# jhuggins/viabel

Measured on AMD Instinct MI355X. Metric: ELBO-gradient evals/sec (D=1024, N_mc=4096), higher is better.
Workload: dtype f64

## Files before the change

viabel_amd/csrc/vb_fullrank.hip:

```cpp
#include "vb_gemm_f64.h"
#include "vb_fit.h"

namespace vb {

constexpr double kLog2PiFr = 1.8378770664093454835606594728112;

__device__ __forceinline__ double fr_wave_sum(double x) {
#pragma unroll
  for (int off = 32; off > 0; off >>= 1) x += __shfl_down(x, off, 64);
  return x;
}

__device__ __forceinline__ double fr_block_sum(double x, double* sh) {
  x = fr_wave_sum(x);
  const int lane = threadIdx.x & 63, wave = threadIdx.x >> 6;
  __syncthreads();
  if (lane == 0) sh[wave] = x;
  __syncthreads();
  return (sh[0] + sh[1]) + (sh[2] + sh[3]);
}

__global__ void __launch_bounds__(256) fr_unpack_kernel(const double* __restrict__ theta, int d,
                                                        int64_t ldl, double* __restrict__ Lt,
                                                        double* __restrict__ mu, double* __restrict__ copy = nullptr) {
// ... 222 lines not shown
    const double v = z[m.k];
    const double w = exp(-2.0 * v);
    const double rw = roww ? roww[row] : 1.0;
    double ss = 0.0;
    for (int c = lane; c < d; c += 64) {
      if (c == m.k) continue;
      const double zc = z[c];
      const double gc = -zc * w;
      g[c] = roww ? gc * rw : gc;
      ss = fma(zc, zc, ss);
    }
    ss = fr_wave_sum(ss);
    if (lane == 0) {
      const double it2 = 1.0 / (m.tau * m.tau), dm1 = (double)(d - 1);
      const double gk = fma(-v, it2, -dm1) + w * ss;
      g[m.k] = roww ? gk * rw : gk;
      f = v * fma(-0.5 * v, it2, -dm1) - 0.5 * w * ss;
    }
  }
  f = fr_block_sum(f, sh);
  if (threadIdx.x == 0) fpart[blockIdx.x] = f;
}

typedef double fr_d2 __attribute__((ext_vector_type(2)));
__global__ void __launch_bounds__(256) fr_colsum_kernel(const double* __restrict__ G,
                                                        const double* __restrict__ Zc, int64_t ldz,
                                                        int64_t n, int d, int fmode,
                                                        const double* __restrict__ ivar,
                                                        double* __restrict__ colpart,
                                                        double* __restrict__ fpart, double scal = 0.0,
                                                        const double* __restrict__ roww = nullptr,
                                                        int square = 0, double* __restrict__ Gscaled = nullptr,
                                                        const double* __restrict__ rs_out = nullptr) {
  __shared__ double sh[4];
  __shared__ fr_d2 cs[4][64];
  const int c = threadIdx.x & 63, q = threadIdx.x >> 6;
  const int col = blockIdx.x * 128 + 2 * c;
  const int64_t r0 = (int64_t)blockIdx.y * 128;
  const int64_t r1 = r0 + 128 < n ? r0 + 128 : n;
  const bool ok0 = col < d, ok1 = col + 1 < d;
  fr_d2 s = (fr_d2){0.0, 0.0};
  double f = 0.0;
  if (ok0) {
    fr_d2 hiv = (fr_d2){0.0, 0.0};
    if (fmode == 1) hiv = (fr_d2){-0.5 / ivar[col], ok1 ? -0.5 / ivar[col + 1] : 0.0};
    for (int64_t rb = r0 + q; rb < r1; rb += 64) {
      fr_d2 g[16], z[16];
      double rw[16], rs[16];
#pragma unroll
      for (int i = 0; i < 16; ++i) {
        const int64_t r = rb + 4 * i < r1 ? rb + 4 * i : r1 - 1;
        g[i] = *reinterpret_cast<const fr_d2*>(G + r * ldz + col);
        z[i] = fmode >= 2 ? *reinterpret_cast<const fr_d2*>(Zc + r * ldz + col) : (fr_d2){0.0, 0.0};
        rw[i] = roww ? roww[r] : 1.0;
        rs[i] = Gscaled ? rs_out[r] : 1.0;
      }
#pragma unroll
      for (int i = 0; i < 16; ++i) {
        const int64_t r = rb + 4 * i;
        const bool in = r < r1;
        if (roww) g[i] *= rw[i];
        if (square) g[i] *= g[i];
        if (!in) g[i] = (fr_d2){0.0, 0.0}, z[i] = (fr_d2){0.0, 0.0};
        if (!ok1) g[i].y = 0.0, z[i].y = 0.0;
        if (Gscaled && in) *reinterpret_cast<fr_d2*>(Gscaled + r * ldz + col) = g[i] * rs[i];
        s += g[i];
        if (fmode == 1) f = fma(hiv.x * g[i].x, g[i].x, fma(hiv.y * g[i].y, g[i].y, f));
        if (fmode == 2) f = fma(0.5 * z[i].x, g[i].x, fma(0.5 * z[i].y, g[i].y, f));
        if (fmode == 3) f = fma(-0.5 * scal * z[i].x, z[i].x, fma(-0.5 * scal * z[i].y, z[i].y, f));
      }
    }
  }
  cs[q][c] = s;
  __syncthreads();
  if (q == 0 && ok0) {
    const fr_d2 tot = (cs[0][c] + cs[1][c]) + (cs[2][c] + cs[3][c]);
    colpart[(int64_t)blockIdx.y * ldz + col] = tot.x;
    if (ok1) colpart[(int64_t)blockIdx.y * ldz + col + 1] = tot.y;
  }
  f = fr_block_sum(f, sh);
  if (threadIdx.x == 0) fpart[(int64_t)blockIdx.y * gridDim.x + blockIdx.x] = f;
}

__global__ void __launch_bounds__(256) fr_fold_ssum_kernel(const double* __restrict__ Spart, int gsplits, int64_t slab, int d,
                                                           int64_t ldl, const double* __restrict__ colpart, int64_t ldz,
                                                           const double* __restrict__ M, const double* __restrict__ P,
                                                           int64_t ldp, const double* __restrict__ mu,
                                                           const double* __restrict__ mean, double n_rows, int nb_cs,
                                                           int nb_s, double* __restrict__ S, double* __restrict__ svec,
                                                           double* __restrict__ b, double* __restrict__ csg) {
  if ((int)blockIdx.x < nb_cs) {
    __shared__ fr_d2 part[2][64][4];
    const int p = threadIdx.x & 3, kg = threadIdx.x >> 2;
    const int col = (int)blockIdx.x * 8 + 2 * p;
    const int colc = col < d ? col : 0;
    const int kper = (d + 63) / 64;
    const int k0 = kg * kper, k1 = k0 + kper < d ? k0 + kper : d;
    fr_d2 acc = (fr_d2){0.0, 0.0}, bacc = (fr_d2){0.0, 0.0};
    for (int kb = k0; kb < k1; kb += 16) {
      fr_d2 v[16];
      double c[16];
#pragma unroll
      for (int u = 0; u < 16; ++u) {
        const int k = kb + u < k1 ? kb + u : k1 - 1;
        v[u] = *reinterpret_cast<const fr_d2*>(P + (int64_t)k * ldp + colc);
        c[u] = mu[k] - mean[k];
      }
#pragma unroll
      for (int u = 0; u < 16; ++u)
        if (kb + u < k1) bacc += v[u] * c[u];
    }
    for (int kb = k0; kb < k1; kb += 16) {
      fr_d2 v[16];
      double c[16];
#pragma unroll
      for (int u = 0; u < 16; ++u) {
        const int k = kb + u < k1 ? kb + u : k1 - 1;
        v[u] = *reinterpret_cast<const fr_d2*>(M + (int64_t)k * ldz + colc);
        c[u] = colpart[k];
      }
      for (int z = 1; z < gsplits; ++z)
#pragma unroll
        for (int u = 0; u < 16; ++u) c[u] += colpart[(int64_t)z * ldz + (kb + u < k1 ? kb + u : k1 - 1)];
#pragma unroll
      for (int u = 0; u < 16; ++u)
        if (kb + u < k1) acc += v[u] * c[u];
    }
    part[0][kg][p] = acc;
    part[1][kg][p] = bacc;
    __syncthreads();
    if (kg == 0) {
      fr_d2 tot = part[0][0][p], btot = part[1][0][p];
#pragma unroll 16
      for (int q = 1; q < 64; ++q) tot += part[0][q][p], btot += part[1][q][p];
      if (col < d) b[col] = btot.x, csg[col] = -tot.x - n_rows * btot.x;
      if (col + 1 < d) b[col + 1] = btot.y, csg[col + 1] = -tot.y - n_rows * btot.y;
    }
    return;
  }
  if ((int)blockIdx.x < nb_cs + nb_s) {
    const int k = ((int)blockIdx.x - nb_cs) * 256 + (int)threadIdx.x;
    if (k >= ldz) return;
    double s = 0.0;
    if (k < d) {
      s = colpart[k];
      for (int z = 1; z < gsplits; ++z) s += colpart[(int64_t)z * ldz + k];
    }
    svec[k] = s;
    return;
  }
  int bi = 0, bj = (int)blockIdx.x - nb_cs - nb_s;
  while (bj > bi) bj -= ++bi;
  __shared__ double tile[32][33];
  const int tx = threadIdx.x & 31, ty = threadIdx.x >> 5;
  const int i0 = bi * 32, j0 = bj * 32;
  double v[4];
  int64_t idx[4];
#pragma unroll
  for (int q = 0; q < 4; ++q) {
    const int i = i0 + ty + 8 * q, j = j0 + tx;
    idx[q] = (i < d && j <= i) ? (int64_t)i * ldl + j : 0;
    v[q] = 0.0;
  }
  for (int zb = 0; zb < gsplits; zb += 8) {
    double w[8][4];
#pragma unroll
    for (int u = 0; u < 8; ++u)
#pragma unroll
      for (int q = 0; q < 4; ++q) w[u][q] = Spart[(zb + u < gsplits ? zb + u : gsplits - 1) * slab + idx[q]];
#pragma unroll
    for (int u = 0; u < 8; ++u)
      if (zb + u < gsplits) {
#pragma unroll
        for (int q = 0; q < 4; ++q) v[q] = (zb + u == 0) ? w[u][q] : v[q] + w[u][q];
      }
  }
#pragma unroll
  for (int q = 0; q < 4; ++q) tile[ty + 8 * q][tx] = v[q];
  __syncthreads();
#pragma unroll
  for (int q = 0; q < 4; ++q) {
    const int r = ty + 8 * q;
    if (bi == bj) {
      const int i = i0 + r, j = j0 + tx;
      if (i < d && j < d) S[(int64_t)i * ldl + j] = tx <= r ? v[q] : tile[tx][r];
    } else {
      const int i = i0 + r, j = j0 + tx;
      if (i < d && j < d) S[(int64_t)i * ldl + j] = v[q];
      const int it = j0 + r, jt = i0 + tx;
      if (it < d && jt < d) S[(int64_t)it * ldl + jt] = tile[tx][r];
    }
  }
}

static int fr_fold_csplits(int d, int n_cu, int max_splits) {
  const GemmArgs sc = gemm_product(nullptr, 0, nullptr, 0, d, d, d, 2);
  const long tiles = gemm_count_blocks(sc, 64, 64);
  int s = d / (16 * kGemmBK);
  if ((long)s * tiles > 4L * n_cu) s = (int)(4L * n_cu / tiles);
  if (s > max_splits) s = max_splits;
  if (s > 16) s = 16;
  return s < 1 ? 1 : s;
}


template <int CHUNK>
__global__ void __launch_bounds__(256) fr_reduce_kernel(const double* __restrict__ Cpart, int splits,
                                                        int64_t slab, int d, int64_t ldl,
                                                        const double* __restrict__ colpart, int n_rb,
                                                        int64_t ldz, const double* __restrict__ fpart,
                                                        int n_fpart, FrSums S, int full,
                                                        const double* __restrict__ wpart, int nb_c) {
  __shared__ double sh[4];
  const int nb_col = (int)((ldz + 255) / 256);
  if ((int)blockIdx.x < nb_c) {
    const int64_t tid = (int64_t)blockIdx.x * 256 + threadIdx.x;
    const int64_t idx = 2 * tid;
    const int64_t nC = (int64_t)d * ldl;
    if (idx >= nC) return;
    const int i = (int)(idx / ldl), j = (int)(idx % ldl);
    fr_d2 s = (fr_d2){0.0, 0.0};
    if (full == 1 || j <= i) {
      for (int k0 = 0; k0 < splits; k0 += CHUNK) {
        fr_d2 v[CHUNK];
#pragma unroll
        for (int u = 0; u < CHUNK; ++u)
          v[u] = *reinterpret_cast<const fr_d2*>(Cpart + (k0 + u < splits ? k0 + u : splits - 1) * slab + idx);
#pragma unroll
        for (int u = 0; u < CHUNK; ++u)
          if (k0 + u < splits) s += v[u];
      }
      if (full != 1 && j + 1 > i) s.y = 0.0;
    }
    if (full == 2) {
      double* C = S.sums + S.off_c;
      if (j < d && j <= i) {
        C[idx] = s.x;
        if (j < i) C[(int64_t)j * ldl + i] = s.x;
      } else if (j >= d) {
        C[idx] = 0.0;
      }
      if (j + 1 < d && j + 1 <= i) {
        C[idx + 1] = s.y;
        if (j + 1 < i) C[(int64_t)(j + 1) * ldl + i] = s.y;
      } else if (j + 1 >= d) {
        C[idx + 1] = 0.0;
      }
    } else {
      *reinterpret_cast<fr_d2*>(S.sums + S.off_c + idx) = s;
    }
    return;
  }
  if ((int)blockIdx.x < nb_c + nb_col) {
    const int64_t tid = (int64_t)((int)blockIdx.x - nb_c) * 256 + threadIdx.x;
    if (tid >= ldz) return;
    double s = 0.0;
    if (tid < d) {
      for (int rb0 = 0; rb0 < n_rb; rb0 += 32) {
        double v[32];
#pragma unroll
        for (int u = 0; u < 32; ++u) v[u] = rb0 + u < n_rb ? colpart[(int64_t)(rb0 + u) * ldz + tid] : 0.0;
#pragma unroll
        for (int u = 0; u < 32; ++u) s += v[u];
      }
    }
    S.sums[S.off_col + tid] = s;
    return;
  }
  double f = 0.0;
  for (int e = threadIdx.x; e < n_fpart; e += 256) f += fpart[e];
  f = fr_block_sum(f, sh);
  if (threadIdx.x == 0) S.sums[0] = f;
  if (wpart) {
    for (int q = 0; q < 2; ++q) {
      double t = 0.0;
// ... 875 lines not shown
static int fr_prepare_dense(vb_ctx* ctx, const FrRoute& r, FrBufs* b, const double* theta_dev) {
  const int64_t d = r.d;
  VB_TRY(ensure(ctx, ctx->fr_lt, (size_t)(r.ldz + r.slab) * sizeof(double)));
  b->mu = (double*)ctx->fr_lt.ptr;
  b->Lt = b->mu + r.ldz;
  const bool resident = theta_dev == (const double*)ctx->fr_theta.ptr;
  const bool stepped = ctx->fr_lt_owner != nullptr && ctx->fr_lt_owner == theta_dev;
  const bool lt_cached = (resident || stepped) && ctx->fr_lt_d == d;
  if (!stepped) ctx->fr_lt_owner = nullptr;
  ctx->fr_lt_d = (resident || stepped) ? d : 0;
  if (!lt_cached) {
    hipLaunchKernelGGL(fr_unpack_kernel, dim3((unsigned)((d + 31) / 32), (unsigned)((d + 31) / 32)), dim3(256), 0, ctx->stream,
                       theta_dev, r.D, r.ldl, b->Lt, b->mu);
    VB_HIP(ctx, hipGetLastError());
  }
  return VB_OK;
}

static int fr_score_prologue(vb_ctx* ctx, const FrRoute& r, const FrBufs& b, const double* theta_dev) {
  hipStream_t st = ctx->stream;
  const int D = r.D;
  VB_TRY(fr_tri_inverse_enqueue(ctx, st, theta_dev, b.Lt, D, r.ldl, b.Xa, b.T));
  VB_HIP(ctx, hipGetLastError());
  hipLaunchKernelGGL(fr_transpose_kernel, dim3((unsigned)((D + 31) / 32), (unsigned)((D + 31) / 32)), dim3(256), 0, st,
                     (const double*)b.Xa, b.T, D, r.ldl);
  const int sq_blocks = (int)(r.n < 256 ? r.n : 256);
  hipLaunchKernelGGL(fr_sumsq_kernel, dim3((unsigned)sq_blocks), dim3(256), 0, st, b.E, b.lde, r.n, D, b.sq);
  hipLaunchKernelGGL(fr_sumsq_final_kernel, dim3(1), dim3(256), 0, st, (const double*)b.sq, sq_blocks, b.S.sums + 1);
  VB_HIP(ctx, hipGetLastError());
  return VB_OK;
}

static GemmArgs fr_sample_product(vb_ctx* ctx, const FrRoute& r, const FrBufs& b) {
  GemmArgs g1 = gemm_product(b.E, b.lde, b.Lt, r.ldl, (int)r.n, r.D, r.D, r.tri1);
  prof_events(ctx, &g1.ev0, &g1.ev1, 1, VB_PROF_FR_SAMPLE_GEMM);
  return g1;
}

static const double* fr_sample(vb_ctx* ctx, const FrRoute& r, const FrBufs& b, const double* shift, const double* row_scale,
                               const double* z_ready) {
  if (r.caller_z) return z_ready;
  hipStream_t st = ctx->stream;
  const GemmArgs g1 = fr_sample_product(ctx, r, b);
  if (r.kparts > 1) {
    gemm_f64_launch<true>(st, g1, r.kparts, r.n_cu, EpiSplitSlab{b.Cpart, r.ldz, r.pslab});
    hipLaunchKernelGGL(fr_zsum_kernel, dim3(r.sum_blocks), dim3(256), 0, st, (const double*)b.Cpart, r.kparts, r.pslab, r.n,
                       r.D, r.ldz, (const double*)b.mu, shift, b.Z);
  } else {
    gemm_f64_launch<true>(st, g1, 1, r.n_cu, EpiStoreZ{b.Z, r.ldz, b.mu, shift, row_scale});
  }
  return b.Z;
}

static unsigned fr_model_gauss_diag(vb_ctx* ctx, const FrRoute& r, const FrBufs& b, const ModelDev& m,
                                    const double* row_scale) {
  const GemmArgs g1 = fr_sample_product(ctx, r, b);
  if (r.diag_f)
    return gemm_f64_launch<true>(ctx->stream, g1, 1, r.n_cu, EpiGaussDiagF{b.G, r.ldz, b.mu, m.p0, m.p1, b.fpart});
  gemm_f64_launch<true>(ctx->stream, g1, 1, r.n_cu, EpiGaussDiag{b.G, r.ldz, b.mu, m.p0, m.p1, row_scale});
  return 0;
}

static int fr_model_funnel(vb_ctx* ctx, const FrRoute& r, const FrBufs& b, const ModelDev& m, const double* Z,
                           const double* roww) {
  hipLaunchKernelGGL(fr_funnel_kernel, dim3((unsigned)((r.n + 3) / 4)), dim3(256), 0, ctx->stream, Z, b.G, r.ldz, r.n, r.D, m,
                     b.fpart, roww);
  return VB_OK;
}

static int fr_model_source(vb_ctx* ctx, const FrRoute& r, const FrBufs& b, const double* Z) {
  return model_rows_enqueue(ctx, ctx->stream, Z, r.ldz, r.n, r.D, b.G, r.ldz, b.fpart);
}

static int fr_model_glm(vb_ctx* ctx, const FrRoute& r, const FrBufs& b, const ModelDev& m, const double* Z) {
  hipStream_t st = ctx->stream;
  double* part = b.fpart + (int64_t)r.n_rb * r.cs_gx;
  VB_HIP(ctx, hipMemsetAsync(part, 0, (size_t)r.glm_part * sizeof(double), st));
  const GemmArgs gh = gemm_product(Z, r.ldz, m.p1, m.ldq, (int)r.n, (int)m.n_data, r.D, 0);
  gemm_f64_launch<true>(st, gh, 1, r.n_cu, EpiGlm{b.Rm, r.ldr, m.p2, part, m.link, m.aux});
  VB_HIP(ctx, hipGetLastError());
  return glm_grad_enqueue(ctx, st, m, b.Rm, r.ldr, Z, b.G, r.ldz, r.n, r.D);
}

static int fr_model_folded(vb_ctx* ctx, const FrRoute& r, const FrBufs& b, const ModelDev& m) {
  hipStream_t st = ctx->stream;
  const int D = r.D;
  const GemmArgs gm = gemm_product(b.Lt, r.ldl, m.p1, m.ldp, D, D, D, 4);
  gemm_f64_launch<true, true>(st, gm, 1, r.n_cu, EpiSplitSlab{b.Mf, r.ldz, r.slab});
  VB_HIP(ctx, hipGetLastError());
  return VB_OK;
}

static int fr_grad_folded(vb_ctx* ctx, const FrRoute& r, const FrBufs& b, const ModelDev& m, unsigned* tiles3) {
  hipStream_t st = ctx->stream;
  const int D = r.D;
  const double* M = b.Mf;
  GemmArgs gs = gemm_product(b.E, b.lde, b.E, b.lde, D, D, (int)r.n, 2);
  prof_events(ctx, &gs.ev0, &gs.ev1, 1, VB_PROF_FR_GRAD_GEMM);
  if (r.cfg3 == 2) VB_TRY(tri2_tile_map(ctx, D, 128, 64, &gs.tile_map, &gs.tile_blocks));
  gemm_f64_launch<false>(st, gs, r.splits, r.n_cu, EpiSplitSlabCs{b.Cpart, r.ldl, r.slab, b.colpart, r.ldz}, r.cfg3);
  VB_HIP(ctx, hipGetLastError());
  const int nb_cs = (D + 7) / 8, nb_s = (int)((r.ldz + 255) / 256), tiles = (D + 31) / 32;
  hipLaunchKernelGGL(fr_fold_ssum_kernel, dim3((unsigned)(nb_cs + nb_s + tiles * (tiles + 1) / 2)), dim3(256), 0, st,
                     (const double*)b.Cpart, r.splits, r.slab, D, r.ldl, (const double*)b.colpart, r.ldz, M, m.p1,
                     (int64_t)m.ldp, (const double*)b.mu, m.p0, (double)r.n, nb_cs, nb_s, b.Sg, b.svec, b.bvec, b.csg);
  VB_HIP(ctx, hipGetLastError());
  GemmArgs gc = gemm_product(M, r.ldz, b.Sg, r.ldl, D, D, D, 2);
  if (r.cfgc == 2) VB_TRY(tri2_tile_map(ctx, D, 128, 64, &gc.tile_map, &gc.tile_blocks));
  *tiles3 = gemm_f64_launch<false>(st, gc, r.csplits, r.n_cu,
                                   EpiFoldSlabF{b.Cpart, r.ldl, r.slab, b.bvec, b.svec, b.Lt, r.ldl, b.fpart}, r.cfgc);
  VB_HIP(ctx, hipGetLastError());
  return VB_OK;
}

static int fr_model_gauss_full(vb_ctx* ctx, const FrRoute& r, const FrBufs& b, const ModelDev& m, const double* row_scale,
                               const double* g_ready, double** G, unsigned* tiles2) {
  hipStream_t st = ctx->stream;
  const int D = r.D;
  *G = b.G;
  GemmArgs g2 = gemm_product(b.Z, r.ldz, m.p1, m.ldp, (int)r.n, D, D, 0);
  switch (r.dense) {
    case kDenseNoG:
      return fr_model_folded(ctx, r, b, m);
    case kDenseCallerG:
      *G = const_cast<double*>(g_ready);
      return VB_OK;
    case kDensePersistent: {
      const GemmArgs g1 = gemm_product(b.E, b.lde, b.Lt, r.ldl, (int)r.n, D, D, r.tri1);
      GemmArgs g3f = gemm_product(b.G, r.ldz, b.E, b.lde, D, D, (int)r.n, 2);
      if (r.fz_mode == 3) VB_TRY(tri2_tile_map(ctx, D, 128, 64, &g3f.tile_map, &g3f.tile_blocks));
      return fr_fused_enqueue(ctx, st, r.fz_mode, g1, g2, g3f, r.splits, b.Z, b.G, r.ldz, b.mu, m.p0, b.fpart,
                              EpiSplitSlabCs{b.Cpart, r.ldl, r.slab, b.colpart, r.ldz}, tiles2);
    }
    case kDenseChain:
      break;
  }
  fr_sample(ctx, r, b, m.p0, row_scale, nullptr);
  VB_HIP(ctx, hipGetLastError());
  if (r.model_ksplit) {
    gemm_f64_launch<true>(st, g2, r.kparts, r.n_cu, EpiSplitSlab{b.Cpart, r.ldz, r.pslab});
    hipLaunchKernelGGL(fr_gsum_kernel, dim3(r.sum_blocks), dim3(256), 0, st, (const double*)b.Cpart, r.kparts, r.pslab, r.n, D,
                       r.ldz, (const double*)b.Z, b.G, b.fpart);
    *tiles2 = r.sum_blocks;
    return VB_OK;
  }
  prof_events(ctx, &g2.ev0, &g2.ev1, 1, VB_PROF_FR_MODEL_GEMM);
  if (r.fused_sums) *tiles2 = gemm_f64_launch<true>(st, g2, 1, r.n_cu, EpiNegateF{b.G, r.ldz, b.Z, b.fpart});
  else gemm_f64_launch<true>(st, g2, 1, r.n_cu, EpiNegate{b.G, r.ldz});
  return VB_OK;
}

static int fr_colpass(vb_ctx* ctx, const FrRoute& r, const FrBufs& b, const ModelDev& m, double* G, const double* Z, int fmode,
                      double* fpart, const double* row_scale) {
  hipLaunchKernelGGL(fr_colsum_kernel, dim3((unsigned)r.cs_gx, (unsigned)r.n_rb), dim3(256), 0, ctx->stream, (const double*)G, Z,
                     r.ldz, r.n, r.D, fmode, m.p1, b.colpart, fpart, r.glm ? 1.0 / (m.tau * m.tau) : 0.0,
                     (const double*)nullptr, 0, row_scale ? G : (double*)nullptr, row_scale);
  VB_HIP(ctx, hipGetLastError());
  return VB_OK;
}

static int fr_rowscale(vb_ctx* ctx, const FrRoute& r, double* G, const double* w) {
  hipLaunchKernelGGL(fr_rowscale_kernel, dim3((unsigned)r.n, (unsigned)((r.D + 255) / 256)), dim3(256), 0, ctx->stream, G, r.ldz,
                     r.n, r.D, w);
  VB_HIP(ctx, hipGetLastError());
  return VB_OK;
}

static int fr_score(vb_ctx* ctx, const FrRoute& r, const FrBufs& b, const ModelDev& m, double* G, const double* Z) {
  if (r.two_passes) VB_TRY(fr_colpass(ctx, r, b, m, G, Z, r.fmode, b.fpart, nullptr));
  const GemmArgs gy = gemm_product(b.E, b.lde, b.T, r.ldl, (int)r.n, r.D, r.D, 3);
  gemm_f64_launch<true>(ctx->stream, gy, 1, r.n_cu, EpiAccumulate{G, r.ldz});
  VB_HIP(ctx, hipGetLastError());
  return VB_OK;
}

static int fr_grad_product(vb_ctx* ctx, const FrRoute& r, const FrBufs& b, const ModelDev& m, const double* G,
                           unsigned* tiles3) {
  hipStream_t st = ctx->stream;
  *tiles3 = 0;
  if (r.fold) return fr_grad_folded(ctx, r, b, m, tiles3);
  if (!r.grad_launch) return VB_OK;
  GemmArgs g3 = gemm_product(G, r.ldz, b.E, b.lde, r.D, r.D, (int)r.n, r.tri3);
  prof_events(ctx, &g3.ev0, &g3.ev1, 1, VB_PROF_FR_GRAD_GEMM);
  if (r.cfg3 == 2) VB_TRY(tri2_tile_map(ctx, r.D, 128, 64, &g3.tile_map, &g3.tile_blocks));
  if (r.grad_colsums)
    *tiles3 = gemm_f64_launch<false>(st, g3, r.splits, r.n_cu, EpiSplitSlabCs{b.Cpart, r.ldl, r.slab, b.colpart, r.ldz}, r.cfg3);
  else
    *tiles3 = gemm_f64_launch<false>(st, g3, r.splits, r.n_cu, EpiSplitSlab{b.Cpart, r.ldl, r.slab});
  VB_HIP(ctx, hipGetLastError());
  return VB_OK;
}

static int fr_finish_mvt(vb_ctx* ctx, const FrRoute& r, const FrBufs& b, FrSums* sums_out) {
  fr_reduce_launch(ctx, ctx->stream, (const double*)b.Cpart, r.splits, r.slab, r.D, r.ldl, (const double*)b.colpart, r.n_rb, r.ldz,
                   (const double*)b.fpart, r.n_fpart, b.S, 1, nullptr);
  VB_HIP(ctx, hipGetLastError());
  if (ctx->comm) VB_TRY(comm_allreduce_sum(ctx, ctx->stream, b.S.sums, (size_t)b.S.len));
  *sums_out = b.S;
  return VB_OK;
}

static int fr_finish_dense(vb_ctx* ctx, const FrRoute& r, const FrBufs& b, const ModelDev& m, int set, int n_fpart_red,
                           const double* theta_dev, double* out_dev, int64_t n_total, const FrWeighted& wm) {
  hipStream_t st = ctx->stream;
  const int D = r.D, n_rb_red = r.fold ? 1 : (r.grad_colsums || !r.grad_launch) ? r.splits : r.n_rb;
  const int splits = r.fold ? r.csplits : r.splits;
// ... 132 lines not shown
```

viabel_amd/csrc/vb_gemm_f64.h:

```cpp
#pragma once

#include "vb_common.h"

#include <cstdlib>
#include <type_traits>
#include <utility>

namespace vb {

typedef double d2v __attribute__((ext_vector_type(2)));
typedef double d4v __attribute__((ext_vector_type(4)));

constexpr int kGemmBK = 16;

#ifdef VB_GEMM_CLOCK
__device__ long long vb_gemm_dbg[8 * 4096];
#endif

struct GemmArgs {
  const double* A = nullptr;
  const double* B = nullptr;
  int64_t lda = 0, ldb = 0;
  int M = 0, N = 0, K = 0;
  int tiles_m = 0, tiles_n = 0;
// ... 194 lines not shown
  if (k_begin < k_end) {
    load_slab(k_begin);
    store_slab(0);
    load_slab(k_begin + kGemmBK);
    __syncthreads();
    load_frags(0, 0, 0);
    int buf = 0;
    for (int k0 = k_begin; k0 < k_end; k0 += kGemmBK) {
#ifndef VB_GEMM_SKIP
#define VB_GEMM_SKIP 0
#endif
      if (!(VB_GEMM_SKIP & 2)) store_slab(buf ^ 1);
      if (!(VB_GEMM_SKIP & 1)) load_slab(k0 + 2 * kGemmBK);
#pragma unroll
      for (int kk = 0; kk < KS - 1; ++kk) {
        if (!(VB_GEMM_SKIP & 8)) load_frags(buf, kk + 1, (kk + 1) & 1);
        mfma_step(kk & 1);
        interleave(kk == 0 ? 1 : (kk == 1 ? 2 : 0));
      }
      if (!(VB_GEMM_SKIP & 4)) __syncthreads();
      if (!(VB_GEMM_SKIP & 8)) load_frags(buf ^ 1, 0, KS & 1);
      mfma_step((KS - 1) & 1);
      interleave(0);
      buf ^= 1;
    }
  }

#ifdef VB_GEMM_CLOCK
  if (t == 0) {
    vb_gemm_dbg[2 * blockIdx.x] = clock64() - dbg_c0;
    vb_gemm_dbg[2 * blockIdx.x + 1] = wall_clock64() - dbg_w0;
  }
#endif
  double local = 0.0;
#pragma unroll
  for (int a = 0; a < AF; ++a)
#pragma unroll
    for (int r = 0; r < NB; ++r) {
      const int row = m0 + wm * (16 * AF) + a * 16 + 4 * fblk + fk;
      const int col = n0 + wn * (4 * NB) + 4 * ((fblk + r) & (NB - 1)) + fj;
      if (row < g.M && col < g.N) {
        if constexpr (EpiReduces<Epi>::value)
          local += epi((int)blockIdx.z, row, col, acc[a][r]);
        else
          epi((int)blockIdx.z, row, col, acc[a][r]);
      }
    }
  if constexpr (EpiReduces<Epi>::value) {
    __syncthreads();
#pragma unroll
    for (int off = 32; off > 0; off >>= 1) local += __shfl_down(local, off, 64);
    double* red = &As[0][0][0];
    if (lane == 0) red[wave] = local;
    __syncthreads();
    if (t == 0) epi.part[(int64_t)blockIdx.z * gridDim.x + blockIdx.x] = (red[0] + red[1]) + (red[2] + red[3]);
  }
}

}

#include "vb_gemm_f64_dma.h"

namespace vb {

inline int gemm_tiles(int x, int b) { return (x + b - 1) / b; }

inline int64_t gemm_max_blocks(int64_t M, int64_t N) { return ((M + 63) / 64) * ((N + 63) / 64); }

inline long gemm_count_blocks(const GemmArgs& g, int bm_rows, int bn_cols) {
  const int tm = gemm_tiles(g.M, bm_rows), tn = gemm_tiles(g.N, bn_cols);
  if (g.tri_mode != 2) return (long)tm * tn;
  long blocks = 0;
  for (int bm = 0; bm < tm; ++bm) {
    const int cnt = (bm * bm_rows + bm_rows - 1) / bn_cols + 1;
    blocks += cnt < tn ? cnt : tn;
  }
  return blocks;
}

inline bool gemm_uses_dma(const GemmArgs& g) {
  return g.K % kGemmBK == 0 && g.M > 0 && g.N > 0;
}

template <bool A_KCONTIG, bool TRI4_PAIRS = false, class Epi>
inline unsigned gemm_f64_launch(hipStream_t st, GemmArgs g, int splits, int n_cu, const Epi& epi, int cfg = 0,
                                int flags = 0) {
  constexpr bool kNarrowOk = A_KCONTIG && !EpiColsum<Epi>::value;
  constexpr bool kNarrowAuto = kNarrowOk && !EpiReduces<Epi>::value && !EpiRowSums<Epi>::value;
  if (splits < 1) splits = 1;
  int ks = g.batch ? g.K : gemm_tiles(g.K, splits);
  g.k_split = gemm_tiles(ks, kGemmBK) * kGemmBK;
  const bool dma = gemm_uses_dma(g) && !(flags & 1);
  if (g.tri_mode == 3 && (!dma || splits != 1 || g.batch)) g.tri_mode = 0;
  if (g.tri_mode == 4 && (!dma || !A_KCONTIG || g.batch)) g.tri_mode = 0;
  if (cfg == 0) {
    if (dma && (g.tri_mode == 1 || g.tri_mode == 3) && splits == 1 && gemm_count_blocks(g, 128, 64) < 4L * n_cu) {
      cfg = 4;
      if (kNarrowAuto && !g.batch && gemm_count_blocks(g, 64, 64) <= 2L * n_cu) cfg = 8;
    } else if (dma && g.tri_mode == 0 && g.batch == 0 && gemm_count_blocks(g, 128, 128) * splits >= 2L * n_cu) {
      cfg = 6;
    } else if (!dma && gemm_count_blocks(g, 128, 128) * splits >= 2L * n_cu) {
      cfg = 1;
    } else if (gemm_count_blocks(g, 128, 64) * splits * 100 >= 190L * n_cu) {
      cfg = 2;
    } else {
      cfg = 3;
      if (kNarrowAuto && dma && g.tri_mode == 0 && !g.batch && gemm_count_blocks(g, 64, 64) * splits <= (long)n_cu) cfg = 7;
    }
  }
  static_assert(!TRI4_PAIRS || kNarrowAuto, "paired row blocks: A[m][k], an epilogue that only stores");
  const bool pairs = TRI4_PAIRS && g.tri_mode == 4 && splits == 1;
  if (pairs) cfg = 7;
  if (!kNarrowOk && cfg >= 7) cfg = 4;
  if (!dma && cfg > 3) cfg = (cfg == 4 || cfg >= 7) ? 3 : cfg == 6 ? 1 : 2;
  const int bm_rows = (cfg == 3 || cfg == 4 || cfg >= 7) ? 64 : 128, bn_cols = cfg >= 7 ? 32 : (cfg == 1 || cfg == 6) ? 128 : 64;
  g.tiles_m = gemm_tiles(g.M, bm_rows);
  g.tiles_n = gemm_tiles(g.N, bn_cols);
  if (splits % 8 != 0 || g.batch) g.xcd_group = 0;
  dim3 grid(g.tile_map ? (unsigned)g.tile_blocks : (unsigned)gemm_count_blocks(g, bm_rows, bn_cols), 1, (unsigned)splits);
  if (pairs) grid = dim3((unsigned)((g.tiles_m + 1) / 2 * g.tiles_n), 1, 1);
  g.prio_div = (g.tri_mode != 1 && g.tri_mode != 3 && g.tri_mode != 4) ? n_cu : 0;
  if (dma) {
    if (cfg == 1) gemm_f64_dma_launch<A_KCONTIG, 4, 16, 3, Epi>(st, g, grid, epi);
    else if (cfg == 2) gemm_f64_dma_launch<A_KCONTIG, 4, 8, 3, Epi>(st, g, grid, epi);
    else if (cfg == 3) gemm_f64_dma_launch<A_KCONTIG, 2, 8, 3, Epi>(st, g, grid, epi);
    else if (cfg == 4) gemm_f64_dma_launch<A_KCONTIG, 2, 8, 2, Epi>(st, g, grid, epi);
    else if (cfg == 6) gemm_f64_dma_launch<A_KCONTIG, 4, 16, 2, Epi>(st, g, grid, epi);
    else if (cfg >= 7) {
      if constexpr (TRI4_PAIRS) {
        if (pairs) {
          gemm_f64_dma_pair_launch<2, 4, 3, Epi>(st, g, grid, epi);
          return grid.x;
        }
      }
      if constexpr (kNarrowOk) {
        if (cfg == 7) gemm_f64_dma_launch<A_KCONTIG, 2, 4, 3, Epi>(st, g, grid, epi);
        else gemm_f64_dma_launch<A_KCONTIG, 2, 4, 2, Epi>(st, g, grid, epi);
      }
    }
    else gemm_f64_dma_launch<A_KCONTIG, 4, 8, 2, Epi>(st, g, grid, epi);
    return grid.x;
  }
  if (cfg == 1)
    hipExtLaunchKernelGGL((gemm_f64_kernel<A_KCONTIG, 4, 16, Epi>), grid, dim3(256), 0, st, g.ev0, g.ev1, 0, g, epi);
  else if (cfg == 2)
    hipExtLaunchKernelGGL((gemm_f64_kernel<A_KCONTIG, 4, 8, Epi>), grid, dim3(256), 0, st, g.ev0, g.ev1, 0, g, epi);
  else
    hipExtLaunchKernelGGL((gemm_f64_kernel<A_KCONTIG, 2, 8, Epi>), grid, dim3(256), 0, st, g.ev0, g.ev1, 0, g, epi);
  return grid.x;
}

}
```

viabel_amd/csrc/vb_gemm_f64_dma.h:

```cpp
#pragma once

namespace vb {

typedef __attribute__((address_space(1))) const void* gemm_gptr;
typedef __attribute__((address_space(3))) void* gemm_lptr;

struct GemmNoDep {
  static constexpr int kAuxA = 0;
  __device__ __forceinline__ void before_slab(int, int, int, bool) const {}
  __device__ __forceinline__ void publish(int, int, int) const {}
};

template <bool A_KCONTIG, int AF, int NB, int STAGES, class Epi, class Dep>
__device__ __forceinline__ void gemm_f64_dma_tile(const GemmArgs& g, const Epi& epi, const Dep& dep, const int bx,
                                                  const int bz, const int gx) {
  constexpr int BM = 32 * AF, BN = 8 * NB;
  constexpr int kStages = STAGES;
  static_assert(STAGES == 2 || STAGES == 3, "two or three LDS stages");
  constexpr int kATile = BM * kGemmBK, kBTile = kGemmBK * BN;
  constexpr int kAUnits = kATile / 128, kBUnits = kBTile / 128;
  constexpr int UPW = (kAUnits + kBUnits) / 4;
  static_assert((kAUnits + kBUnits) % 4 == 0, "units must divide over the 4 waves");
  extern __shared__ double gemm_lds[];
  double* As = gemm_lds;
// ... 350 lines not shown
      s.x += __shfl_xor(s.x, 1, 64), s.y += __shfl_xor(s.y, 1, 64);
      s.x += __shfl_xor(s.x, 2, 64), s.y += __shfl_xor(s.y, 2, 64);
      if (fj == 0) rsum[wn * BM + lrow] = s;
    }
    __syncthreads();
    if (t < BM && m0 + t < g.M) epi.rows_out(m0 + t, bn, rsum[t] + rsum[BM + t]);
    dep.publish(bm, bn, bz);
    return;
  }
#pragma unroll
  for (int a = 0; a < AF; ++a)
#pragma unroll
    for (int r = 0; r < NB; r += 2) {
      const int row = m0 + frag_row(a, 4 * fblk + fk);
      const int col = n0 + frag_col(r, fblk, fj);
      if constexpr (EpiPairs<Epi>::value && AF * NB <= 32) {
        if (row < g.M && col + 1 < g.N) {
          const d2v v = epi.pair((int)bz, row, col, acc[a][r], acc[a][r + 1]);
          if constexpr (EpiReduces<Epi>::value) {
            local += v.x;
            local += v.y;
          }
          continue;
        }
      }
#pragma unroll
      for (int q = 0; q < 2; ++q) {
        if (row < g.M && col + q < g.N) {
          if constexpr (EpiReduces<Epi>::value)
            local += epi((int)bz, row, col + q, acc[a][r + q]);
          else
            epi((int)bz, row, col + q, acc[a][r + q]);
        }
      }
    }
  if constexpr (EpiReduces<Epi>::value) {
#pragma unroll
    for (int off = 32; off > 0; off >>= 1) local += __shfl_down(local, off, 64);
    if (lane == 0) gemm_lds[wave] = local;
    __syncthreads();
    if (t == 0)
      epi.part[(int64_t)bz * gx + bx] = (gemm_lds[0] + gemm_lds[1]) + (gemm_lds[2] + gemm_lds[3]);
  }
  dep.publish(bm, bn, bz);
#ifdef VB_GEMM_CLOCK
  __builtin_amdgcn_s_waitcnt(0);
  if (lane == 0 && bx < 1024) {
    long long* o = vb_gemm_dbg + 8 * (4 * bx + wave);
    o[0] = dbg_t1 - dbg_t0;
    o[1] = dbg_t2 - dbg_t1;
    o[2] = clock64() - dbg_t2;
    o[3] = wall_clock64() - dbg_w0;
    o[4] = dbg_w0;
  }
#endif
}


template <bool A_KCONTIG, int AF, int NB, int STAGES, class Epi>
__global__ void __launch_bounds__(256, AF * NB > 32 ? (STAGES > 2 ? 1 : 2) : (AF * NB > 16 || STAGES > 2 ? 2 : 4))
    gemm_f64_dma_kernel(const GemmArgs g, const Epi epi) {
  int bx = (int)blockIdx.x, bz = (int)blockIdx.z;
  if (g.xcd_group) {
    const unsigned lin = blockIdx.x + gridDim.x * blockIdx.z, slot = lin >> 3;
    bz = (int)((lin & 7) + 8 * (slot / gridDim.x));
    bx = (int)(slot % gridDim.x);
  }
  gemm_f64_dma_tile<A_KCONTIG, AF, NB, STAGES, Epi, GemmNoDep>(g, epi, GemmNoDep{}, bx, bz, (int)gridDim.x);
}

template <bool A_KCONTIG, int AF, int NB, int STAGES, class Epi>
inline void gemm_f64_dma_launch(hipStream_t st, const GemmArgs& g, dim3 grid, const Epi& epi) {
  constexpr size_t lds = (size_t)STAGES * (32 * AF * kGemmBK + kGemmBK * 8 * NB) * sizeof(double);
  static bool configured = false;
  if (!configured) {
    (void)hipFuncSetAttribute(reinterpret_cast<const void*>(&gemm_f64_dma_kernel<A_KCONTIG, AF, NB, STAGES, Epi>),
                              hipFuncAttributeMaxDynamicSharedMemorySize, (int)lds);
    configured = true;
  }
  hipExtLaunchKernelGGL((gemm_f64_dma_kernel<A_KCONTIG, AF, NB, STAGES, Epi>), grid, dim3(256), lds, st, g.ev0, g.ev1,
                        0, g, epi);
}

struct GemmPairNoDep : GemmNoDep {};

template <int AF, int NB, int STAGES, class Epi>
__global__ void __launch_bounds__(256, AF * NB > 32 ? (STAGES > 2 ? 1 : 2) : (AF * NB > 16 || STAGES > 2 ? 2 : 4))
    gemm_f64_dma_pair_kernel(const GemmArgs g, const Epi epi) {
  static_assert(!EpiReduces<Epi>::value && !EpiColsum<Epi>::value && !EpiRowSums<Epi>::value,
                "the epilogue between the passes must leave LDS alone");
  const int pair = (int)blockIdx.x / g.tiles_n, bn = (int)blockIdx.x % g.tiles_n;
  const int mirror = g.tiles_m - 1 - pair;
  const int passes = mirror > pair ? 2 : 1;
#pragma unroll 1
  for (int pass = 0; pass < passes; ++pass) {
    const int bm = pass == 0 ? pair : mirror;
    const int bx = bm * g.tiles_n + bn, bz = 0;
    gemm_f64_dma_tile<true, AF, NB, STAGES, Epi, GemmPairNoDep>(g, epi, GemmPairNoDep{}, bx, bz, (int)gridDim.x);
    __asm__ volatile("" ::: "memory");
    __builtin_amdgcn_s_waitcnt(0);
    __asm__ volatile("" ::: "memory");
  }
}

template <int AF, int NB, int STAGES, class Epi>
inline void gemm_f64_dma_pair_launch(hipStream_t st, const GemmArgs& g, dim3 grid, const Epi& epi) {
  constexpr size_t lds = (size_t)STAGES * (32 * AF * kGemmBK + kGemmBK * 8 * NB) * sizeof(double);
  static bool configured = false;
  if (!configured) {
    (void)hipFuncSetAttribute(reinterpret_cast<const void*>(&gemm_f64_dma_pair_kernel<AF, NB, STAGES, Epi>),
                              hipFuncAttributeMaxDynamicSharedMemorySize, (int)lds);
    configured = true;
  }
  hipExtLaunchKernelGGL((gemm_f64_dma_pair_kernel<AF, NB, STAGES, Epi>), grid, dim3(256), lds, st, g.ev0, g.ev1, 0, g, epi);
}

}
```

Before: 5740.

## Fuse folded M-product GEMM into fold-sum kernel and split csg into C-tile launch

The folded path previously launched the Lt·P1 product (M) as a separate paired GEMM, then a fold kernel that computed b, svec, symmetric S and csg (which reads M). Now the M-product tiles run as extra blocks inside the fold-sum kernel alongside the b/svec/S blocks. The csg column reduction, which depends on M, moves to a later launch, either fused as extra blocks into the C-product GEMM kernel (cfgc 4) or as its own small kernel. This removes a launch and overlaps independent work, at the cost of sharing dynamic LDS sizing and mixing heterogeneous blocks in one grid.

```diff
diff --git a/viabel_amd/csrc/vb_fullrank.hip b/viabel_amd/csrc/vb_fullrank.hip
--- a/viabel_amd/csrc/vb_fullrank.hip
+++ b/viabel_amd/csrc/vb_fullrank.hip
@@ -328,21 +328,29 @@
   if (threadIdx.x == 0) fpart[(int64_t)blockIdx.y * gridDim.x + blockIdx.x] = f;
 }
 
-__global__ void __launch_bounds__(256) fr_fold_ssum_kernel(const double* __restrict__ Spart, int gsplits, int64_t slab, int d,
+struct FoldMsumNoDep : GemmNoDep {};
+
+__global__ void __launch_bounds__(256) fr_fold_msum_kernel(const GemmArgs gm, const EpiSplitSlab em, int nb_m,
+                                                           const double* __restrict__ Spart, int gsplits, int64_t slab, int d,
                                                            int64_t ldl, const double* __restrict__ colpart, int64_t ldz,
-                                                           const double* __restrict__ M, const double* __restrict__ P,
-                                                           int64_t ldp, const double* __restrict__ mu,
-                                                           const double* __restrict__ mean, double n_rows, int nb_cs,
-                                                           int nb_s, double* __restrict__ S, double* __restrict__ svec,
-                                                           double* __restrict__ b, double* __restrict__ csg) {
-  if ((int)blockIdx.x < nb_cs) {
-    __shared__ fr_d2 part[2][64][4];
+                                                           const double* __restrict__ P, int64_t ldp,
+                                                           const double* __restrict__ mu, const double* __restrict__ mean,
+                                                           int nb_b, int nb_s, double* __restrict__ S,
+                                                           double* __restrict__ svec, double* __restrict__ b) {
+  extern __shared__ double fold_lds[];
+  if ((int)blockIdx.x < nb_m) {
+    gemm_f64_dma_pair_tiles<2, 4, 3, EpiSplitSlab, FoldMsumNoDep>(gm, em, FoldMsumNoDep{}, (int)blockIdx.x, nb_m);
+    return;
+  }
+  const int blk = (int)blockIdx.x - nb_m;
+  if (blk < nb_b) {
+    fr_d2(*part)[4] = reinterpret_cast<fr_d2(*)[4]>(fold_lds);
     const int p = threadIdx.x & 3, kg = threadIdx.x >> 2;
-    const int col = (int)blockIdx.x * 8 + 2 * p;
+    const int col = blk * 8 + 2 * p;
     const int colc = col < d ? col : 0;
     const int kper = (d + 63) / 64;
     const int k0 = kg * kper, k1 = k0 + kper < d ? k0 + kper : d;
-    fr_d2 acc = (fr_d2){0.0, 0.0}, bacc = (fr_d2){0.0, 0.0};
+    fr_d2 bacc = (fr_d2){0.0, 0.0};
     for (int kb = k0; kb < k1; kb += 16) {
       fr_d2 v[16];
       double c[16];
@@ -356,36 +364,19 @@
       for (int u = 0; u < 16; ++u)
         if (kb + u < k1) bacc += v[u] * c[u];
     }
-    for (int kb = k0; kb < k1; kb += 16) {
-      fr_d2 v[16];
-      double c[16];
-#pragma unroll
-      for (int u = 0; u < 16; ++u) {
-        const int k = kb + u < k1 ? kb + u : k1 - 1;
-        v[u] = *reinterpret_cast<const fr_d2*>(M + (int64_t)k * ldz + colc);
-        c[u] = colpart[k];
-      }
-      for (int z = 1; z < gsplits; ++z)
-#pragma unroll
-        for (int u = 0; u < 16; ++u) c[u] += colpart[(int64_t)z * ldz + (kb + u < k1 ? kb + u : k1 - 1)];
-#pragma unroll
-      for (int u = 0; u < 16; ++u)
-        if (kb + u < k1) acc += v[u] * c[u];
-    }
-    part[0][kg][p] = acc;
-    part[1][kg][p] = bacc;
+    part[kg][p] = bacc;
     __syncthreads();
     if (kg == 0) {
-      fr_d2 tot = part[0][0][p], btot = part[1][0][p];
+      fr_d2 btot = part[0][p];
 #pragma unroll 16
-      for (int q = 1; q < 64; ++q) tot += part[0][q][p], btot += part[1][q][p];
-      if (col < d) b[col] = btot.x, csg[col] = -tot.x - n_rows * btot.x;
-      if (col + 1 < d) b[col + 1] = btot.y, csg[col + 1] = -tot.y - n_rows * btot.y;
+      for (int q = 1; q < 64; ++q) btot += part[q][p];
+      if (col < d) b[col] = btot.x;
+      if (col + 1 < d) b[col + 1] = btot.y;
     }
     return;
   }
-  if ((int)blockIdx.x < nb_cs + nb_s) {
-    const int k = ((int)blockIdx.x - nb_cs) * 256 + (int)threadIdx.x;
+  if (blk < nb_b + nb_s) {
+    const int k = (blk - nb_b) * 256 + (int)threadIdx.x;
     if (k >= ldz) return;
     double s = 0.0;
     if (k < d) {
@@ -395,9 +386,9 @@
     svec[k] = s;
     return;
   }
-  int bi = 0, bj = (int)blockIdx.x - nb_cs - nb_s;
+  int bi = 0, bj = blk - nb_b - nb_s;
   while (bj > bi) bj -= ++bi;
-  __shared__ double tile[32][33];
+  double(*tile)[33] = reinterpret_cast<double(*)[33]>(fold_lds);
   const int tx = threadIdx.x & 31, ty = threadIdx.x >> 5;
   const int i0 = bi * 32, j0 = bj * 32;
   double v[4];
@@ -437,6 +428,67 @@
       if (it < d && jt < d) S[(int64_t)it * ldl + jt] = tile[tx][r];
     }
   }
+}
+
+template <int U>
+__device__ __forceinline__ void fr_fold_csg_blocks(const int blk, fr_d2 (*part)[4], const double* __restrict__ colpart,
+                                                   int gsplits, int64_t ldz, int d, const double* __restrict__ M,
+                                                   const double* __restrict__ b, double n_rows, double* __restrict__ csg) {
+  const int p = threadIdx.x & 3, kg = threadIdx.x >> 2;
+  const int col = blk * 8 + 2 * p;
+  const int colc = col < d ? col : 0;
+  const int kper = (d + 63) / 64;
+  const int k0 = kg * kper, k1 = k0 + kper < d ? k0 + kper : d;
+  fr_d2 acc = (fr_d2){0.0, 0.0};
+  for (int kb = k0; kb < k1; kb += U) {
+    fr_d2 v[U];
+    double c[U];
+#pragma unroll
+    for (int u = 0; u < U; ++u) {
+      const int k = kb + u < k1 ? kb + u : k1 - 1;
+      v[u] = *reinterpret_cast<const fr_d2*>(M + (int64_t)k * ldz + colc);
+      c[u] = colpart[k];
+    }
+    for (int z = 1; z < gsplits; ++z)
+#pragma unroll
+      for (int u = 0; u < U; ++u) c[u] += colpart[(int64_t)z * ldz + (kb + u < k1 ? kb + u : k1 - 1)];
+#pragma unroll
+    for (int u = 0; u < U; ++u)
+      if (kb + u < k1) acc += v[u] * c[u];
+  }
+  part[kg][p] = acc;
+  __syncthreads();
+  if (kg == 0) {
+    fr_d2 tot = part[0][p];
+#pragma unroll 16
+    for (int q = 1; q < 64; ++q) tot += part[q][p];
+    if (col < d) csg[col] = -tot.x - n_rows * b[col];
+    if (col + 1 < d) csg[col + 1] = -tot.y - n_rows * b[col + 1];
+  }
+}
+
+__global__ void __launch_bounds__(256) fr_fold_csg_kernel(const double* __restrict__ colpart, int gsplits, int64_t ldz, int d,
+                                                          const double* __restrict__ M, const double* __restrict__ b,
+                                                          double n_rows, double* __restrict__ csg) {
+  __shared__ fr_d2 part[64][4];
+  fr_fold_csg_blocks<16>((int)blockIdx.x, part, colpart, gsplits, ldz, d, M, b, n_rows, csg);
+}
+
+struct FoldCsgNoDep : GemmNoDep {};
+
+__global__ void __launch_bounds__(256, 4) fr_fold_ctile_csg_kernel(const GemmArgs g, const EpiFoldSlabF epi, int gx, int nb_tiles,
+                                                                   const double* __restrict__ colpart, int gsplits, int64_t ldz,
+                                                                   int d, const double* __restrict__ M,
+                                                                   const double* __restrict__ b, double n_rows,
+                                                                   double* __restrict__ csg) {
+  if ((int)blockIdx.x < nb_tiles) {
+    const int bz = (int)blockIdx.x / gx, bx = (int)blockIdx.x - bz * gx;
+    gemm_f64_dma_tile<false, 2, 8, 2, EpiFoldSlabF, FoldCsgNoDep>(g, epi, FoldCsgNoDep{}, bx, bz, gx);
+    return;
+  }
+  extern __shared__ double fold_lds[];
+  fr_fold_csg_blocks<8>((int)blockIdx.x - nb_tiles, reinterpret_cast<fr_d2(*)[4]>(fold_lds), colpart, gsplits, ldz, d, M, b,
+                        n_rows, csg);
 }
 
 static int fr_fold_csplits(int d, int n_cu, int max_splits) {
@@ -1478,15 +1530,6 @@
   return glm_grad_enqueue(ctx, st, m, b.Rm, r.ldr, Z, b.G, r.ldz, r.n, r.D);
 }
 
-static int fr_model_folded(vb_ctx* ctx, const FrRoute& r, const FrBufs& b, const ModelDev& m) {
-  hipStream_t st = ctx->stream;
-  const int D = r.D;
-  const GemmArgs gm = gemm_product(b.Lt, r.ldl, m.p1, m.ldp, D, D, D, 4);
-  gemm_f64_launch<true, true>(st, gm, 1, r.n_cu, EpiSplitSlab{b.Mf, r.ldz, r.slab});
-  VB_HIP(ctx, hipGetLastError());
-  return VB_OK;
-}
-
 static int fr_grad_folded(vb_ctx* ctx, const FrRoute& r, const FrBufs& b, const ModelDev& m, unsigned* tiles3) {
   hipStream_t st = ctx->stream;
   const int D = r.D;
@@ -1496,15 +1539,47 @@
   if (r.cfg3 == 2) VB_TRY(tri2_tile_map(ctx, D, 128, 64, &gs.tile_map, &gs.tile_blocks));
   gemm_f64_launch<false>(st, gs, r.splits, r.n_cu, EpiSplitSlabCs{b.Cpart, r.ldl, r.slab, b.colpart, r.ldz}, r.cfg3);
   VB_HIP(ctx, hipGetLastError());
+  GemmArgs gm = gemm_product(b.Lt, r.ldl, m.p1, m.ldp, D, D, D, 4);
+  const unsigned nb_m = gemm_f64_pair_plan(&gm);
+  if (nb_m == 0) return fail(ctx, VB_ERR_STATE, "folded evaluation: D = %d does not go to the LDS-DMA product", D);
   const int nb_cs = (D + 7) / 8, nb_s = (int)((r.ldz + 255) / 256), tiles = (D + 31) / 32;
-  hipLaunchKernelGGL(fr_fold_ssum_kernel, dim3((unsigned)(nb_cs + nb_s + tiles * (tiles + 1) / 2)), dim3(256), 0, st,
-                     (const double*)b.Cpart, r.splits, r.slab, D, r.ldl, (const double*)b.colpart, r.ldz, M, m.p1,
-                     (int64_t)m.ldp, (const double*)b.mu, m.p0, (double)r.n, nb_cs, nb_s, b.Sg, b.svec, b.bvec, b.csg);
+  constexpr size_t msum_lds = gemm_f64_dma_pair_lds<2, 4, 3>();
+  static_assert(msum_lds >= 64 * 4 * sizeof(fr_d2) && msum_lds >= 32 * 33 * sizeof(double), "the sum blocks' LDS is the tiles'");
+  static bool configured = false;
+  if (!configured) {
+    (void)hipFuncSetAttribute(reinterpret_cast<const void*>(&fr_fold_msum_kernel), hipFuncAttributeMaxDynamicSharedMemorySize,
+                              (int)msum_lds);
+    configured = true;
+  }
+  hipLaunchKernelGGL(fr_fold_msum_kernel, dim3(nb_m + (unsigned)(nb_cs + nb_s + tiles * (tiles + 1) / 2)), dim3(256), msum_lds, st,
+                     gm, EpiSplitSlab{b.Mf, r.ldz, r.slab}, (int)nb_m, (const double*)b.Cpart, r.splits, r.slab, D, r.ldl,
+                     (const double*)b.colpart, r.ldz, m.p1, (int64_t)m.ldp, (const double*)b.mu, m.p0, nb_cs, nb_s, b.Sg, b.svec,
+                     b.bvec);
   VB_HIP(ctx, hipGetLastError());
   GemmArgs gc = gemm_product(M, r.ldz, b.Sg, r.ldl, D, D, D, 2);
+  const EpiFoldSlabF ec{b.Cpart, r.ldl, r.slab, b.bvec, b.svec, b.Lt, r.ldl, b.fpart};
+  if (r.cfgc == 4) {
+    const int gx = (int)gemm_f64_tri2_small_plan(&gc, r.csplits, r.n_cu), nb_tiles = gx * r.csplits;
+    if (gx == 0) return fail(ctx, VB_ERR_STATE, "folded evaluation: D = %d does not go to the LDS-DMA product", D);
+    constexpr size_t lds = (size_t)2 * (64 * kGemmBK + kGemmBK * 64) * sizeof(double);
+    static_assert(lds >= 64 * 4 * sizeof(fr_d2), "the colsum(G) blocks' LDS is the tiles'");
+    static bool configured_c = false;
+    if (!configured_c) {
+      (void)hipFuncSetAttribute(reinterpret_cast<const void*>(&fr_fold_ctile_csg_kernel), hipFuncAttributeMaxDynamicSharedMemorySize,
+                                (int)lds);
+      configured_c = true;
+    }
+    hipLaunchKernelGGL(fr_fold_ctile_csg_kernel, dim3((unsigned)(nb_tiles + nb_cs)), dim3(256), lds, st, gc, ec, gx, nb_tiles,
+                       (const double*)b.colpart, r.splits, r.ldz, D, M, (const double*)b.bvec, (double)r.n, b.csg);
+    VB_HIP(ctx, hipGetLastError());
+    *tiles3 = (unsigned)gx;
+    return VB_OK;
+  }
   if (r.cfgc == 2) VB_TRY(tri2_tile_map(ctx, D, 128, 64, &gc.tile_map, &gc.tile_blocks));
-  *tiles3 = gemm_f64_launch<false>(st, gc, r.csplits, r.n_cu,
-                                   EpiFoldSlabF{b.Cpart, r.ldl, r.slab, b.bvec, b.svec, b.Lt, r.ldl, b.fpart}, r.cfgc);
+  *tiles3 = gemm_f64_launch<false>(st, gc, r.csplits, r.n_cu, ec, r.cfgc);
+  VB_HIP(ctx, hipGetLastError());
+  hipLaunchKernelGGL(fr_fold_csg_kernel, dim3((unsigned)nb_cs), dim3(256), 0, st, (const double*)b.colpart, r.splits, r.ldz, D, M,
+                     (const double*)b.bvec, (double)r.n, b.csg);
   VB_HIP(ctx, hipGetLastError());
   return VB_OK;
 }
@@ -1517,7 +1592,7 @@
   GemmArgs g2 = gemm_product(b.Z, r.ldz, m.p1, m.ldp, (int)r.n, D, D, 0);
   switch (r.dense) {
     case kDenseNoG:
-      return fr_model_folded(ctx, r, b, m);
+      return VB_OK;
     case kDenseCallerG:
       *G = const_cast<double*>(g_ready);
       return VB_OK;
diff --git a/viabel_amd/csrc/vb_gemm_f64.h b/viabel_amd/csrc/vb_gemm_f64.h
--- a/viabel_amd/csrc/vb_gemm_f64.h
+++ b/viabel_amd/csrc/vb_gemm_f64.h
@@ -300,7 +300,27 @@
   return g.K % kGemmBK == 0 && g.M > 0 && g.N > 0;
 }
 
-template <bool A_KCONTIG, bool TRI4_PAIRS = false, class Epi>
+inline unsigned gemm_f64_pair_plan(GemmArgs* g) {
+  if (g->tri_mode != 4 || g->batch || !gemm_uses_dma(*g)) return 0;
+  g->k_split = gemm_tiles(g->K, kGemmBK) * kGemmBK;
+  g->tiles_m = gemm_tiles(g->M, 64);
+  g->tiles_n = gemm_tiles(g->N, 32);
+  g->xcd_group = 0;
+  g->prio_div = 0;
+  return (unsigned)((g->tiles_m + 1) / 2 * g->tiles_n);
+}
+
+inline unsigned gemm_f64_tri2_small_plan(GemmArgs* g, int splits, int n_cu) {
+  if (g->tri_mode != 2 || g->batch || g->tile_map || splits < 1 || !gemm_uses_dma(*g)) return 0;
+  g->k_split = gemm_tiles(gemm_tiles(g->K, splits), kGemmBK) * kGemmBK;
+  g->tiles_m = gemm_tiles(g->M, 64);
+  g->tiles_n = gemm_tiles(g->N, 64);
+  g->xcd_group = 0;
+  g->prio_div = n_cu;
+  return (unsigned)gemm_count_blocks(*g, 64, 64);
+}
+
+template <bool A_KCONTIG, class Epi>
 inline unsigned gemm_f64_launch(hipStream_t st, GemmArgs g, int splits, int n_cu, const Epi& epi, int cfg = 0,
                                 int flags = 0) {
   constexpr bool kNarrowOk = A_KCONTIG && !EpiColsum<Epi>::value;
@@ -326,9 +346,6 @@
       if (kNarrowAuto && dma && g.tri_mode == 0 && !g.batch && gemm_count_blocks(g, 64, 64) * splits <= (long)n_cu) cfg = 7;
     }
   }
-  static_assert(!TRI4_PAIRS || kNarrowAuto, "paired row blocks: A[m][k], an epilogue that only stores");
-  const bool pairs = TRI4_PAIRS && g.tri_mode == 4 && splits == 1;
-  if (pairs) cfg = 7;
   if (!kNarrowOk && cfg >= 7) cfg = 4;
   if (!dma && cfg > 3) cfg = (cfg == 4 || cfg >= 7) ? 3 : cfg == 6 ? 1 : 2;
   const int bm_rows = (cfg == 3 || cfg == 4 || cfg >= 7) ? 64 : 128, bn_cols = cfg >= 7 ? 32 : (cfg == 1 || cfg == 6) ? 128 : 64;
@@ -336,7 +353,6 @@
   g.tiles_n = gemm_tiles(g.N, bn_cols);
   if (splits % 8 != 0 || g.batch) g.xcd_group = 0;
   dim3 grid(g.tile_map ? (unsigned)g.tile_blocks : (unsigned)gemm_count_blocks(g, bm_rows, bn_cols), 1, (unsigned)splits);
-  if (pairs) grid = dim3((unsigned)((g.tiles_m + 1) / 2 * g.tiles_n), 1, 1);
   g.prio_div = (g.tri_mode != 1 && g.tri_mode != 3 && g.tri_mode != 4) ? n_cu : 0;
   if (dma) {
     if (cfg == 1) gemm_f64_dma_launch<A_KCONTIG, 4, 16, 3, Epi>(st, g, grid, epi);
@@ -345,12 +361,6 @@
     else if (cfg == 4) gemm_f64_dma_launch<A_KCONTIG, 2, 8, 2, Epi>(st, g, grid, epi);
     else if (cfg == 6) gemm_f64_dma_launch<A_KCONTIG, 4, 16, 2, Epi>(st, g, grid, epi);
     else if (cfg >= 7) {
-      if constexpr (TRI4_PAIRS) {
-        if (pairs) {
-          gemm_f64_dma_pair_launch<2, 4, 3, Epi>(st, g, grid, epi);
-          return grid.x;
-        }
-      }
       if constexpr (kNarrowOk) {
         if (cfg == 7) gemm_f64_dma_launch<A_KCONTIG, 2, 4, 3, Epi>(st, g, grid, epi);
         else gemm_f64_dma_launch<A_KCONTIG, 2, 4, 2, Epi>(st, g, grid, epi);
diff --git a/viabel_amd/csrc/vb_gemm_f64_dma.h b/viabel_amd/csrc/vb_gemm_f64_dma.h
--- a/viabel_amd/csrc/vb_gemm_f64_dma.h
+++ b/viabel_amd/csrc/vb_gemm_f64_dma.h
@@ -456,37 +456,28 @@
                         0, g, epi);
 }
 
-struct GemmPairNoDep : GemmNoDep {};
-
-template <int AF, int NB, int STAGES, class Epi>
-__global__ void __launch_bounds__(256, AF * NB > 32 ? (STAGES > 2 ? 1 : 2) : (AF * NB > 16 || STAGES > 2 ? 2 : 4))
-    gemm_f64_dma_pair_kernel(const GemmArgs g, const Epi epi) {
+template <int AF, int NB, int STAGES, class Epi, class Dep>
+__device__ __forceinline__ void gemm_f64_dma_pair_tiles(const GemmArgs& g, const Epi& epi, const Dep& dep, const int block,
+                                                        const int gx) {
   static_assert(!EpiReduces<Epi>::value && !EpiColsum<Epi>::value && !EpiRowSums<Epi>::value,
                 "the epilogue between the passes must leave LDS alone");
-  const int pair = (int)blockIdx.x / g.tiles_n, bn = (int)blockIdx.x % g.tiles_n;
+  const int pair = block / g.tiles_n, bn = block % g.tiles_n;
   const int mirror = g.tiles_m - 1 - pair;
   const int passes = mirror > pair ? 2 : 1;
 #pragma unroll 1
   for (int pass = 0; pass < passes; ++pass) {
     const int bm = pass == 0 ? pair : mirror;
     const int bx = bm * g.tiles_n + bn, bz = 0;
-    gemm_f64_dma_tile<true, AF, NB, STAGES, Epi, GemmPairNoDep>(g, epi, GemmPairNoDep{}, bx, bz, (int)gridDim.x);
+    gemm_f64_dma_tile<true, AF, NB, STAGES, Epi, Dep>(g, epi, dep, bx, bz, gx);
     __asm__ volatile("" ::: "memory");
     __builtin_amdgcn_s_waitcnt(0);
     __asm__ volatile("" ::: "memory");
   }
 }
 
-template <int AF, int NB, int STAGES, class Epi>
-inline void gemm_f64_dma_pair_launch(hipStream_t st, const GemmArgs& g, dim3 grid, const Epi& epi) {
-  constexpr size_t lds = (size_t)STAGES * (32 * AF * kGemmBK + kGemmBK * 8 * NB) * sizeof(double);
-  static bool configured = false;
-  if (!configured) {
-    (void)hipFuncSetAttribute(reinterpret_cast<const void*>(&gemm_f64_dma_pair_kernel<AF, NB, STAGES, Epi>),
-                              hipFuncAttributeMaxDynamicSharedMemorySize, (int)lds);
-    configured = true;
-  }
-  hipExtLaunchKernelGGL((gemm_f64_dma_pair_kernel<AF, NB, STAGES, Epi>), grid, dim3(256), lds, st, g.ev0, g.ev1, 0, g, epi);
-}
-
-}
+template <int AF, int NB, int STAGES>
+constexpr size_t gemm_f64_dma_pair_lds() {
+  return (size_t)STAGES * (32 * AF * kGemmBK + kGemmBK * 8 * NB) * sizeof(double);
+}
+
+}
```

Result: faster. 6181, median of 6 (+7.7%).
